# rbesenczi/newMSM

Measured on AMD Instinct MI355X. Metric: label-cost evals/sec, higher is better.
Workload: dtype f64; 1 GPU; pairwise sulc (D=1) unary label-cost table, ico6 data grid / ico4 control grid, 19 labels, 48678 evals = 3187573 point samples per step (BASELINE config 2); kind=univariate, simmeasure=correlation, replicas=1

## Files before the change

include/msmhip.h:

```cpp
#ifndef MSMHIP_H
#define MSMHIP_H

#include <stddef.h>
#include <stdint.h>

#ifdef __cplusplus
extern "C" {
#endif

#define MSM_ABI_VERSION 12

#define MSM_OK 0
#define MSM_ERR_INVALID (-1)
#define MSM_ERR_HIP (-2)
#define MSM_ERR_OUTSIDE (-3)
#define MSM_ERR_NOTFOUND (-4)
#define MSM_ERR_NOGPU (-5)
#define MSM_ERR_STATE (-6)
#define MSM_ERR_CAPACITY (-7)
#define MSM_ERR_ROTATION (-8)

#define MSM_RAD 100.0
#define MSM_FOLDING 1e7

typedef struct msm_ctx msm_ctx;
typedef struct msm_mesh msm_mesh;
typedef struct msm_cost msm_cost;

int         msm_abi_version(void);
const char *msm_last_error(void);
int         msm_device_count(void);

int msm_icosphere_counts(int order, int32_t *V, int32_t *T);
int msm_icosphere(int order, double radius, double *xyz, int32_t *tri);
int msm_mesh_adjacency(const int32_t *tri, int32_t V, int32_t T, int32_t *nbr_ptr, int32_t *nbr, int32_t *tid_ptr, int32_t *tid);
int msm_vertex_areas(const double *xyz, const int32_t *tri, int32_t V, int32_t T, double *area);
int msm_resample_anatomy_grid(const double *cp_xyz, int32_t N, const int32_t *cp_tri, int32_t Tc, int32_t levels, double rad, int32_t *Va, int32_t *Ta,
                              double *axyz, int32_t *atri, int32_t *w_ptr, int32_t *w_cp, double *w_val, int32_t *face_ptr, int32_t *face_idx);
int msm_cp_spacings(const double *xyz, const int32_t *tri, int32_t V, int32_t T, double *maxsep, double *mvdmax);
int msm_label_sampling_grid(int sg_order, double max_dist, int abs_is_int, int32_t cap,
                            double *samples, int32_t *nsamples, double *barycentres, int32_t *nbarycentres);
int msm_rescale_sampling_grid(const double *samples, int32_t n, double *scale, double *labels);
int msm_rotation_matrix(const double ci[3], const double index[3], double R[9]);
int msm_cp_rotations(const double centre[3], const double *cp_xyz, int32_t N, double *rot);
int msm_estimate_triplets(const int32_t *tri, int32_t T, int32_t *triplets);
int msm_estimate_pairs(const int32_t *tri, int32_t V, int32_t T, int32_t *pairs);
int msm_octree_signature(const double *xyz, const int32_t *tri, int32_t V, int32_t T, int64_t stats[5], uint64_t *signature);
int msm_ray_table_check(const double *xyz, const int32_t *tri, int32_t V, int32_t T, int32_t nsamples, uint64_t seed, int64_t report[10]);
int msm_ray_hint_check(const double *xyz, const int32_t *tri, int32_t V, int32_t T, int32_t nsamples, uint64_t seed, int64_t report[8], int32_t *cells,
                       int64_t cells_cap);
int msm_ray_cert_check(const double *xyz, const int32_t *tri, int32_t V, int32_t T, int32_t nsamples, uint64_t seed, int64_t report[8], int32_t *cells,
                       int64_t cells_cap);
int msm_ray_table_signature(const double *xyz, const int32_t *tri, int32_t V, int32_t T, uint64_t out[13]);

msm_ctx *msm_ctx_create(int device);
msm_ctx *msm_ctx_create_on_stream(int device, void *hip_stream);
void     msm_ctx_destroy(msm_ctx *ctx);
int      msm_ctx_synchronize(msm_ctx *ctx);
void    *msm_ctx_stream(msm_ctx *ctx);
void     msm_store_release_i64(int64_t *addr, int64_t value);
int64_t  msm_load_acquire_i64(const int64_t *addr);
int64_t  msm_min_acquire_i64(const int64_t *addr, int32_t n);
int      msm_ctx_wait_stream(msm_ctx *ctx, void *hip_stream);
int      msm_ctx_staging_stats(msm_ctx *ctx, int64_t out[4]);
int      msm_ctx_time_queries(msm_ctx *ctx, int enable);
int      msm_ctx_query_kernel_ms(msm_ctx *ctx, double *ms);
int      msm_query_lanes(int64_t n_queries);
void    *msm_host_alloc(msm_ctx *ctx, size_t bytes);
void     msm_host_free(msm_ctx *ctx, void *p);
int      msm_host_register(msm_ctx *ctx, void *p, size_t bytes);

msm_mesh *msm_mesh_create(msm_ctx *ctx, const double *xyz, int32_t V, const int32_t *tri, int32_t T);
void      msm_mesh_destroy(msm_mesh *m);
int       msm_mesh_update_coords(msm_mesh *m, const double *xyz);
int       msm_mesh_get_coords(msm_mesh *m, double *xyz);
int       msm_mesh_set_features(msm_mesh *m, const double *feat, int32_t D);
int       msm_mesh_sizes(const msm_mesh *m, int32_t *V, int32_t *T, int32_t *D);
int       msm_mesh_octree_stats(msm_mesh *m, int64_t stats[5]);
int       msm_mesh_octree_signature(msm_mesh *m, int64_t stats[5], uint64_t *signature);
int       msm_octree_forest_signatures(msm_ctx *ctx, const double *xyz, int32_t V, const int32_t *tri, int32_t T, int32_t B, uint64_t *signatures);
int       msm_mesh_prepare_search(msm_mesh *m, int wait, int32_t *ready);

#define MSM_WEIGHTS_PROJECTED 0
#define MSM_WEIGHTS_RAW 1
int msm_query_triangles(msm_mesh *target, const double *q_xyz, int32_t N, int32_t *tri_id, int32_t *v_id, double *w, int weight_mode);
int msm_closest_vertex(msm_mesh *target, const double *q_xyz, int32_t N, int32_t *v_id);
int msm_adaptive_barycentric_weights(msm_mesh *in_mesh, msm_mesh *new_mesh, const double *excl,
                                     int32_t *row_ptr, int32_t *col, double *val, int64_t cap, int64_t *nnz);
int msm_metric_resample(msm_mesh *in_mesh, const double *data, int32_t D, msm_mesh *new_mesh, const double *excl, double *out, double *excl_out);
int msm_sphere_project_warp(msm_mesh *from, const double *to_xyz, double *sphere_xyz, int32_t N);
int msm_mesh_sphere_project_warp(msm_mesh *sphere, msm_mesh *from, const double *to_xyz);
int msm_barycentric_coords_resample(msm_mesh *from, const double *coords_xyz, const double *q_xyz, int32_t N, double *out_xyz);
int msm_smooth_data(msm_mesh *orig, const double *data, int32_t D, msm_mesh *sphlow, double sigma, const double *excl, double *out, double *excl_out);
int msm_nearest_neighbour(msm_mesh *orig, const double *data, int32_t D, const double *q_xyz, int32_t N, const double *excl, double *out, double *excl_out);
int msm_create_exclusion(const double *data, int32_t D, int32_t V, double thrl, double thru, double *excl);

typedef struct msm_resample_plan msm_resample_plan;
#define MSM_RESAMPLE_ADAP_BARY   0
#define MSM_RESAMPLE_BARYCENTRIC 1
#define MSM_RESAMPLE_NEAREST     2
#define MSM_RESAMPLE_SMOOTH      3
#define MSM_F64 0
#define MSM_F32 1
// ... 256 lines not shown
```

newmsm_amd/_lib.py:

```python
import ctypes as C
import os

_HERE = os.path.dirname(os.path.abspath(__file__))
LIB_PATH = os.environ.get("MSM_LIB_PATH") or os.path.join(_HERE, "libmsmhip.so")

c_dp = C.POINTER(C.c_double)
c_ip = C.POINTER(C.c_int32)
c_lp = C.POINTER(C.c_int64)

MSM_OK = 0
ERR_NAMES = {-1: "MSM_ERR_INVALID", -2: "MSM_ERR_HIP", -3: "MSM_ERR_OUTSIDE", -4: "MSM_ERR_NOTFOUND", -5: "MSM_ERR_NOGPU",
             -6: "MSM_ERR_STATE", -7: "MSM_ERR_CAPACITY", -8: "MSM_ERR_ROTATION"}


class MsmError(RuntimeError):

    def __init__(self, code, message):
        super().__init__("%s (%d): %s" % (ERR_NAMES.get(code, "MSM_ERR"), code, message))
        self.code = code


class GroupParams(C.Structure):
    _fields_ = [("simmeasure", C.c_int32), ("fixnan", C.c_int32), ("lambda_", C.c_double), ("mu", C.c_double),
                ("kappa", C.c_double), ("k_exp", C.c_double), ("rexp", C.c_double), ("range", C.c_double), ("percentile", C.c_double)]


class CostParams(C.Structure):
    _fields_ = [("kind", C.c_int32), ("simmeasure", C.c_int32), ("rmode", C.c_int32), ("reserved", C.c_int32),
                ("lambda_", C.c_double), ("mu", C.c_double), ("kappa", C.c_double), ("k_exp", C.c_double),
                ("rexp", C.c_double), ("range", C.c_double), ("percentile", C.c_double)]


class LevelFeaturesParams(C.Structure):
    _fields_ = [("exclude", C.c_int32), ("intensity", C.c_int32), ("varnorm", C.c_int32), ("reserved", C.c_int32), ("thrl", C.c_double), ("thru", C.c_double)]


_VP = C.c_void_p
SIGNATURES = {
    "msm_abi_version": (C.c_int, []),
    "msm_last_error": (C.c_char_p, []),
    "msm_device_count": (C.c_int, []),
    "msm_icosphere_counts": (C.c_int, [C.c_int, c_ip, c_ip]),
    "msm_icosphere": (C.c_int, [C.c_int, C.c_double, c_dp, c_ip]),
    "msm_mesh_adjacency": (C.c_int, [c_ip, C.c_int32, C.c_int32, c_ip, c_ip, c_ip, c_ip]),
    "msm_vertex_areas": (C.c_int, [c_dp, c_ip, C.c_int32, C.c_int32, c_dp]),
    "msm_resample_anatomy_grid": (C.c_int, [c_dp, C.c_int32, c_ip, C.c_int32, C.c_int32, C.c_double, c_ip, c_ip, c_dp, c_ip, c_ip, c_ip, c_dp, c_ip, c_ip]),
    "msm_cp_spacings": (C.c_int, [c_dp, c_ip, C.c_int32, C.c_int32, c_dp, c_dp]),
    "msm_label_sampling_grid": (C.c_int, [C.c_int, C.c_double, C.c_int, C.c_int32, c_dp, c_ip, c_dp, c_ip]),
    "msm_rescale_sampling_grid": (C.c_int, [c_dp, C.c_int32, c_dp, c_dp]),
    "msm_rotation_matrix": (C.c_int, [c_dp, c_dp, c_dp]),
    "msm_cp_rotations": (C.c_int, [c_dp, c_dp, C.c_int32, c_dp]),
    "msm_estimate_triplets": (C.c_int, [c_ip, C.c_int32, c_ip]),
    "msm_estimate_pairs": (C.c_int, [c_ip, C.c_int32, C.c_int32, c_ip]),
    "msm_octree_signature": (C.c_int, [c_dp, c_ip, C.c_int32, C.c_int32, C.POINTER(C.c_int64), C.POINTER(C.c_uint64)]),
    "msm_ray_table_check": (C.c_int, [c_dp, c_ip, C.c_int32, C.c_int32, C.c_int32, C.c_uint64, C.POINTER(C.c_int64)]),
    "msm_ray_hint_check": (C.c_int, [c_dp, c_ip, C.c_int32, C.c_int32, C.c_int32, C.c_uint64, C.POINTER(C.c_int64), c_ip, C.c_int64]),
    "msm_ray_cert_check": (C.c_int, [c_dp, c_ip, C.c_int32, C.c_int32, C.c_int32, C.c_uint64, C.POINTER(C.c_int64), c_ip, C.c_int64]),
    "msm_ray_table_signature": (C.c_int, [c_dp, c_ip, C.c_int32, C.c_int32, C.POINTER(C.c_uint64)]),
    "msm_ctx_create": (_VP, [C.c_int]),
    "msm_ctx_create_on_stream": (_VP, [C.c_int, _VP]),
    "msm_ctx_destroy": (None, [_VP]),
    "msm_ctx_synchronize": (C.c_int, [_VP]),
    "msm_ctx_stream": (_VP, [_VP]),
    "msm_store_release_i64": (None, [_VP, C.c_int64]),
    "msm_load_acquire_i64": (C.c_int64, [_VP]),
    "msm_min_acquire_i64": (C.c_int64, [_VP, C.c_int32]),
    "msm_ctx_time_queries": (C.c_int, [_VP, C.c_int]),
    "msm_ctx_query_kernel_ms": (C.c_int, [_VP, c_dp]),
    "msm_query_lanes": (C.c_int, [C.c_int64]),
    "msm_group_context": (_VP, [_VP]),
    "msm_ctx_wait_stream": (C.c_int, [_VP, _VP]),
    "msm_ctx_staging_stats": (C.c_int, [_VP, C.POINTER(C.c_int64)]),
    "msm_host_alloc": (_VP, [_VP, C.c_size_t]),
    "msm_host_free": (None, [_VP, _VP]),
    "msm_host_register": (C.c_int, [_VP, _VP, C.c_size_t]),
    "msm_mesh_create": (_VP, [_VP, c_dp, C.c_int32, c_ip, C.c_int32]),
    "msm_mesh_destroy": (None, [_VP]),
    "msm_mesh_update_coords": (C.c_int, [_VP, c_dp]),
    "msm_mesh_get_coords": (C.c_int, [_VP, c_dp]),
    "msm_mesh_set_features": (C.c_int, [_VP, c_dp, C.c_int32]),
    "msm_mesh_sizes": (C.c_int, [_VP, c_ip, c_ip, c_ip]),
    "msm_mesh_octree_stats": (C.c_int, [_VP, c_lp]),
    "msm_mesh_octree_signature": (C.c_int, [_VP, c_lp, C.POINTER(C.c_uint64)]),
    "msm_octree_forest_signatures": (C.c_int, [_VP, c_dp, C.c_int32, c_ip, C.c_int32, C.c_int32, C.POINTER(C.c_uint64)]),
    "msm_query_triangles": (C.c_int, [_VP, c_dp, C.c_int32, c_ip, c_ip, c_dp, C.c_int]),
    "msm_closest_vertex": (C.c_int, [_VP, c_dp, C.c_int32, c_ip]),
    "msm_adaptive_barycentric_weights": (C.c_int, [_VP, _VP, c_dp, c_ip, c_ip, c_dp, C.c_int64, c_lp]),
    "msm_metric_resample": (C.c_int, [_VP, c_dp, C.c_int32, _VP, c_dp, c_dp, c_dp]),
    "msm_create_exclusion": (C.c_int, [c_dp, C.c_int32, C.c_int32, C.c_double, C.c_double, c_dp]),
    "msm_resample_plan_create": (_VP, [_VP, _VP, C.c_int, c_dp]),
    "msm_resample_plan_create_smooth": (_VP, [_VP, _VP, C.c_double, c_dp]),
    "msm_resample_plan_divisors": (C.c_int, [_VP, c_dp]),
    "msm_resample_plan_destroy": (None, [_VP]),
    "msm_resample_plan_sizes": (C.c_int, [_VP, c_ip, c_ip, c_lp, c_ip]),
    "msm_resample_plan_weights": (C.c_int, [_VP, c_ip, c_ip, c_dp, C.c_int64]),
    "msm_resample_plan_apply": (C.c_int, [_VP, _VP, C.c_int, C.c_int64, _VP, c_dp]),
    "msm_resample_plan_apply_dev": (C.c_int, [_VP, _VP, C.c_int, C.c_int64, _VP]),
    "msm_resample_plan_apply_labels": (C.c_int, [_VP, c_ip, C.c_int64, C.c_int32, c_ip]),
    "msm_sphere_project_warp": (C.c_int, [_VP, c_dp, c_dp, C.c_int32]),
    "msm_mesh_sphere_project_warp": (C.c_int, [_VP, _VP, c_dp]),
    "msm_barycentric_coords_resample": (C.c_int, [_VP, c_dp, c_dp, C.c_int32, c_dp]),
    "msm_smooth_data": (C.c_int, [_VP, c_dp, C.c_int32, _VP, C.c_double, c_dp, c_dp, c_dp]),
    "msm_mesh_unfold": (C.c_int, [_VP, C.c_double, c_ip, c_ip]),
    "msm_mesh_prepare_search": (C.c_int, [_VP, C.c_int, c_ip]),
    "msm_variance_normalise": (C.c_int, [c_dp, C.c_int32, C.c_int32, c_dp]),
    "msm_histogram_match": (C.c_int, [_VP, C.c_int32, C.c_int32, C.c_int32, c_dp, c_dp, C.c_int32, C.c_int32, c_dp, c_dp, C.c_int32, c_dp]),
    "msm_level_features": (C.c_int, [_VP, C.c_int32, C.POINTER(_VP), C.POINTER(c_dp), C.c_int32, c_dp, C.POINTER(LevelFeaturesParams), c_dp, c_dp]),
    "msm_mcmc_optimise": (C.c_int, [c_dp, c_dp, c_ip, C.c_int32, C.c_int32, C.c_int32, C.c_double, C.c_int32, C.c_uint64, c_ip]),
    "msm_mcmc_optimise_gpu": (C.c_int, [_VP, c_dp, c_dp, c_ip, C.c_int32, C.c_int32, C.c_int32, C.c_double, C.c_int32, C.c_uint64, c_ip]),
# ... 144 lines not shown
```

newmsm_amd/api.py:

```python
import ctypes as C

import numpy as np

from ._lib import CostParams, LevelFeaturesParams, MsmError, c_dp, c_ip, c_lp, check, lib

WEIGHTS_PROJECTED = 0
WEIGHTS_RAW = 1
KINDS = dict(univariate=0, multivariate=1, patchwise=2, ho_univariate=3, ho_multivariate=4)


def _soa(points):
    a = np.ascontiguousarray(np.asarray(points, dtype=np.float64).reshape(-1, 3).T)
    return a, a.ctypes.data_as(c_dp)


def _aos(soa, n):
    return np.ascontiguousarray(np.asarray(soa).reshape(3, n).T)


def _tri_soa(tri):
    a = np.ascontiguousarray(np.asarray(tri, dtype=np.int32).reshape(-1, 3).T)
    return a, a.ctypes.data_as(c_ip)


# ... 63 lines not shown
                                        b.ctypes.data_as(c_dp), C.byref(nb)))
    return np.ascontiguousarray(s[:, : ns.value].T), np.ascontiguousarray(b[:, : nb.value].T)


def rescale_sampling_grid(samples, scale):
    s, ps = _soa(samples)
    n = s.shape[1]
    out = np.zeros((3, n))
    sc = C.c_double(scale)
    check(lib().msm_rescale_sampling_grid(ps, n, C.byref(sc), out.ctypes.data_as(c_dp)))
    return np.ascontiguousarray(out.T), sc.value


def estimate_rotation_matrix(ci, index):
    R = np.zeros(9)
    check(lib().msm_rotation_matrix(_d(ci)[1], _d(index)[1], R.ctypes.data_as(c_dp)))
    return R.reshape(3, 3)


def cp_rotations(centre, cp_xyz):
    x, px = _soa(cp_xyz)
    rot = np.zeros((x.shape[1], 9))
    check(lib().msm_cp_rotations(_d(centre)[1], px, x.shape[1], rot.ctypes.data_as(c_dp)))
    return rot


def octree_signature(xyz, tri):
    x, px = _soa(xyz)
    t, pt = _tri_soa(tri)
    stats = (C.c_int64 * 5)()
    sig = C.c_uint64(0)
    check(lib().msm_octree_signature(px, pt, x.shape[1], t.shape[1], stats, C.byref(sig)))
    return dict(nodes=stats[0], leaves=stats[1], depth=stats[2], refs=stats[3], max_leaf=stats[4]), sig.value


def ray_table_check(xyz, tri, nsamples=20000, seed=1):
    x, px = _soa(xyz)
    t, pt = _tri_soa(tri)
    rep = (C.c_int64 * 10)()
    check(lib().msm_ray_table_check(px, pt, x.shape[1], t.shape[1], nsamples, seed, rep))
    return dict(points=rep[0], by_float=rep[1], by_fp64=rep[2], open=rep[3], violations=rep[4], unusable=rep[5], with_exclusions=rep[6], simple=bool(rep[7]), boxes_checked=rep[8], refused_by_boxes=rep[9])


def ray_hint_check(xyz, tri, nsamples=20000, seed=1, return_cells=False):
    x, px = _soa(xyz)
    t, pt = _tri_soa(tri)
    rep = (C.c_int64 * 8)()
    cells = np.zeros((6 * 512 * 512, 4), dtype=np.int32) if return_cells else None
    check(lib().msm_ray_hint_check(px, pt, x.shape[1], t.shape[1], nsamples, seed, rep, cells.ctypes.data_as(c_ip) if return_cells else None, cells.size if return_cells else 0))
    out = dict(points=rep[0], hinted=rep[1], unhinted=rep[2], listed=rep[3], cells_changed=rep[4], cells=rep[5], cells_with_more=rep[6], subcells=rep[7])
    if return_cells:
        out["cell_array"] = cells[: rep[5]].copy()
    return out


def ray_cert_check(xyz, tri, nsamples=20000, seed=1, return_cells=False):
    x, px = _soa(xyz)
    t, pt = _tri_soa(tri)
    rep = (C.c_int64 * 8)()
    cells = np.zeros((6 * 512 * 512, 4), dtype=np.int32) if return_cells else None
    check(lib().msm_ray_cert_check(px, pt, x.shape[1], t.shape[1], nsamples, seed, rep, cells.ctypes.data_as(c_ip) if return_cells else None, cells.size if return_cells else 0))
    out = dict(points=rep[0], certified_points=rep[1], fp64_failures=rep[2], reference_disagrees=rep[3], subcells=rep[4], certified_subcells=rep[5], cells=rep[6], placed=rep[7])
    if return_cells:
        out["cell_array"] = cells[: rep[6]].copy()
    return out


def ray_table_signature(xyz, tri):
    x, px = _soa(xyz)
    t, pt = _tri_soa(tri)
    out = (C.c_uint64 * 13)()
    check(lib().msm_ray_table_signature(px, pt, x.shape[1], t.shape[1], out))
    names = ("G", "simple", "certs", "cells", "edges", "more", "excl", "r2lo_bits", "r2hi_bits", "cell_hash", "edge_hash", "more_hash", "excl_hash")
    return dict(zip(names, (int(v) for v in out)))


def estimate_triplets(tri):
    t, pt = _tri_soa(tri)
    out = np.zeros((t.shape[1], 3), dtype=np.int32)
    check(lib().msm_estimate_triplets(pt, t.shape[1], out.ctypes.data_as(c_ip)))
    return out


def estimate_pairs(tri, V):
    t, pt = _tri_soa(tri)
    n = lib().msm_estimate_pairs(pt, V, t.shape[1], None)
    if n < 0:
        check(n)
    out = np.zeros((n, 2), dtype=np.int32)
    lib().msm_estimate_pairs(pt, V, t.shape[1], out.ctypes.data_as(c_ip))
    return out


class Context:

    def __init__(self, device=0, stream=None):
        L = lib()
        self.h = L.msm_ctx_create(device) if stream is None else L.msm_ctx_create_on_stream(device, C.c_void_p(stream))
        if not self.h:
            raise MsmError(-5, L.msm_last_error().decode())
        self.device = device

    def synchronize(self):
        check(lib().msm_ctx_synchronize(self.h))

    @property
# ... 1217 lines not shown
```

newmsm_amd/csrc/ray_table_check.cpp:

```cpp
#include <algorithm>
#include <cmath>
#include <cstring>

#include "ray_table.hpp"
#include "search_device.hpp"

namespace msm {

namespace {

struct TableUnderTest {
    const char *hook = "";
    const double *xyz = nullptr;
    const int32_t *tri = nullptr;
    int V = 0, T = 0;
    FlatOctree o;
    DevTree dt{};
    uint64_t rs = 0;
    std::vector<int> hits;

    int build(const char *hook_, const double *xyz_, const int32_t *tri_, int32_t V_, int32_t T_, int32_t nsamples, uint64_t seed, int64_t *report, int nreport) {
        hook = hook_, xyz = xyz_, tri = tri_, V = V_, T = T_;
        if (!xyz || !tri || !report || V <= 0 || T <= 0 || nsamples < 0) return fail(MSM_ERR_INVALID, "%s: bad arguments", hook);
        for (int64_t i = 0; i < 3 * (int64_t)T; ++i)
// ... 140 lines not shown
    return MSM_OK;
}

extern "C" int msm_ray_hint_check(const double *xyz, const int32_t *tri, int32_t V, int32_t T, int32_t nsamples, uint64_t seed, int64_t report[8], int32_t *cells,
                                  int64_t cells_cap) {
    using namespace msm;
    TableUnderTest u;
    MSM_TRY(u.build("msm_ray_hint_check", xyz, tri, V, T, nsamples, seed, report, 8));
    const FlatOctree &o = u.o;
    const DevTree &dt = u.dt;
    report[7] = kRayHintK;
    if (o.rays.G <= 0) return MSM_OK;
    const size_t ncell = o.rays.cell.size();
    report[5] = (int64_t)ncell;
    MSM_TRY(u.copy_cells(cells, cells_cap));
    for (size_t c = 0; c < ncell; ++c) {
        const int4 raw = o.rays.cell[c], ids = ray_cell_ids(raw);
        if (ids.x >= 0 && ids.w < -1) ++report[6];
        const int stored[4] = {ids.x, ids.y, ids.z, ids.w};
        bool same = true;
        for (int k = 0; k < 4; ++k) same = same && stored[k] < T && (stored[k] >= -1 || (k == 3 && -2 - stored[k] < (int)o.rays.more.size()));
        for (int su = 0; su < kRayHintK && same; ++su)
            for (int sv = 0; sv < kRayHintK && same; ++sv) {
                const int h = ray_cell_hint(raw, su, sv);
                const int4 d = ray_cell_first(raw, h);
                const int got[4] = {d.x, d.y, d.z, d.w};
                same = got[0] == stored[h] && (stored[0] < 0 || got[0] >= 0);
                for (int k = 0, j = 1; k < 4; ++k)
                    if (k != h) same = same && got[j++] == stored[k];
            }
        if (!same) ++report[4];
    }
    for (int it = 0; it < nsamples; ++it) {
        const V3 p = scale(normalized(u.random_direction()), kRad);
        ++report[0];
        const std::vector<int> &hits = u.first_pass(p);
        if (hits.size() != 1) continue;
        const int answer = hits[0];
        float fx, fy, fz;
        size_t at;
        int su, sv;
        if (!ray_cell_at(dt, p, fx, fy, fz, at, su, sv)) continue;
        const int4 first = ray_cell_of(dt, p, fx, fy, fz), ids = ray_cell_ids(o.rays.cell[at]);
        if (first.x == answer) ++report[1];
        if (ids.x == answer) ++report[2];
        int4 more = make_int4(ids.w, -1, -1, -1);
        if (ids.x >= 0 && ids.w < -1) more = o.rays.more[-2 - ids.w];
        const int list[7] = {ids.x, ids.y, ids.z, more.x, more.y, more.z, more.w};
        for (int k = 0; k < 7; ++k)
            if (list[k] == answer) {
                ++report[3];
                break;
            }
    }
    return MSM_OK;
}

extern "C" int msm_ray_cert_check(const double *xyz, const int32_t *tri, int32_t V, int32_t T, int32_t nsamples, uint64_t seed, int64_t report[8], int32_t *cells,
                                  int64_t cells_cap) {
    using namespace msm;
    TableUnderTest u;
    MSM_TRY(u.build("msm_ray_cert_check", xyz, tri, V, T, nsamples, seed, report, 8));
    const FlatOctree &o = u.o;
    const DevTree &dt = u.dt;
    if (o.rays.G <= 0) return MSM_OK;
    const size_t ncell = o.rays.cell.size();
    report[6] = (int64_t)ncell;
    MSM_TRY(u.copy_cells(cells, cells_cap));
    for (size_t c = 0; c < ncell; ++c)
        for (int su = 0; su < kRayHintK; ++su)
            for (int sv = 0; sv < kRayHintK; ++sv) {
                ++report[4];
                if (ray_cell_cert(o.rays.cell[c], su, sv)) ++report[5];
            }
    auto rnd = [&]() { return u.rnd(); };
    const int G = o.rays.G;
    auto on_face = [&](int f, double uu, double v) {
        const int a = f >> 1;
        double comp[3];
        comp[a] = (f & 1) ? -1.0 : 1.0, comp[(a + 1) % 3] = uu, comp[(a + 2) % 3] = v;
        return mk(comp[0], comp[1], comp[2]);
    };
    auto check = [&](V3 p) {
        p = scale(normalized(p), kRad);
        ++report[0];
        float fx, fy, fz;
        bool cert;
        const int4 first = ray_cell_of(dt, p, fx, fy, fz, cert);
        if (!cert) return;
        ++report[1];
        const int t = first.x;
        if (t < 0 || t >= T) {
            ++report[2], ++report[3];
            return;
        }
        if (!ray_accepts_fp64(u.vert(t, 0), u.vert(t, 1), u.vert(t, 2), p, norm(p), (double)o.rays.edge[3 * (size_t)t].w - kRayFloatAllowance + 1e-12)) ++report[2];
        const std::vector<int> &hits = u.first_pass(p);
        if (!(hits.size() == 1 && hits[0] == t)) ++report[3];
    };
    for (int it = 0; it < nsamples; ++it) check(u.random_direction());
    const int64_t before = report[0];
    const double cellw = 2.0 / G;
    auto nudge = [&]() { return rnd() < 0.2 ? 0.0 : (rnd() < 0.5 ? -1.0 : 1.0) * 1e-6 * rnd() * cellw; };
    auto border = [&](bool cell_border) {
        const int i = (int)(rnd() * G) % G, s = cell_border ? 0 : 1 + (int)(rnd() * (kRayHintK - 1)) % std::max(1, kRayHintK - 1);
        return -1 + 2.0 * (i + (double)s / kRayHintK) / G + nudge();
// ... 46 lines not shown
```

newmsm_amd/csrc/unary_kernels.hip:

```cpp
#include "search_device.hpp"
#include "similarity_device.hpp"
#include "unary.hpp"

namespace msm {

namespace {

constexpr int kDeferred = 1 << 20;
constexpr unsigned kInvalidPair = 0xffffffffu;

__device__ __forceinline__ void raise_status(int *status, int code) { atomicMin(status, code); }

struct SamplesArgs {
    DevTree tree;
    const double *tfeat;
    int tD;
    int N, L;
    const double *rnl;
    const double *src;
    int Nsrc;
    const int *pptr, *pidx;
    const int *order;
    int pmax;
    int nsplit;
    double *tval;
    int *stri;
    double *sw3;
    unsigned long long *fix_list;
    double *fix_pt;
    unsigned int *fix_cnt;
    const unsigned int *fix_off;
    const double *sfeat;
    const double *cfw;
    const double *absw;
    int simmeasure;
    double percentile;
    double *U;
    int *redo_list;
    unsigned int *redo_count;
    int *status;
};

__device__ __forceinline__ int fast_div(int s, int P, float invP) {
    int q = (int)((float)s * invP);
    if (q * P > s) --q;
    else if ((q + 1) * P <= s) ++q;
    return q;
}

__device__ __forceinline__ double emit_sample(const SamplesArgs &a, size_t g, const V3 &p, int t) {
    const TriRec &r = a.tree.rec[t];
    double wa, wb, wc;
    area_weights(rec_v0(r), rec_v1(r), rec_v2(r), p, wa, wb, wc);
    if (a.tval) {
        const double v = wa * a.tfeat[(size_t)r.id[0] * a.tD] + wb * a.tfeat[(size_t)r.id[1] * a.tD] + wc * a.tfeat[(size_t)r.id[2] * a.tD];
        a.tval[g] = v;
        return v;
    } else {
        a.stri[g] = t;
        a.sw3[3 * g] = wa;
        a.sw3[3 * g + 1] = wb;
        a.sw3[3 * g + 2] = wc;
    }
    return 0.0;
}

__device__ __forceinline__ void emit_failure(const SamplesArgs &a, size_t g, int code) {
    raise_status(a.status, code);
    const double nan = __longlong_as_double(0x7ff8000000000000ll);
    if (a.tval) {
        a.tval[g] = nan;
    } else {
        a.stri[g] = code;
        a.sw3[3 * g] = a.sw3[3 * g + 1] = a.sw3[3 * g + 2] = nan;
    }
}

}

__global__ __launch_bounds__(256) void k_unary_samples(SamplesArgs a) {
    extern __shared__ __align__(16) double lds[];
    double *sx = lds, *sy = sx + a.pmax, *sz = sy + a.pmax;
    double *sA = sz + a.pmax;
    double *sR = sA + 2 * a.pmax;
    double *sT = sR + 9 * a.L;
    unsigned *queue = reinterpret_cast<unsigned *>(sT + (size_t)unary_labels_per_workgroup(a.L, a.nsplit) * a.pmax);
    int *nin = reinterpret_cast<int *>(queue + kQueueCap);
    int *win = nin + kChunk;
    __shared__ int s_qn, s_ndefer;
    const int tid = threadIdx.x, lane = tid & 63;

    {
        int at, l_beg, l_end;
        if (!unary_workgroup_share(blockIdx.x, a.N, a.L, a.nsplit, at, l_beg, l_end)) return;
        const int node = a.order[at];
        const int beg = a.pptr[node], P = a.pptr[node + 1] - beg;
        const size_t gbase = (size_t)a.L * beg;
        for (int i = tid; i < P; i += 256) {
            const int s = a.pidx[beg + i];
            sx[i] = a.src[s];
            sy[i] = a.src[a.Nsrc + s];
            sz[i] = a.src[2 * a.Nsrc + s];
            if (a.U) sA[i] = a.sfeat[s];
        }
        for (int k = tid; k < 9 * a.L; k += 256) sR[k] = a.rnl[(size_t)node * a.L * 9 + k];
        if (tid == 0) s_ndefer = 0;
        const int sbeg = l_beg * P, send = l_end * P;
        const float invP = 1.0f / (float)max(P, 1);

        for (int base = sbeg; base < send; base += kChunk) {
            const int nchunk = min(kChunk, send - base);
            for (int k = tid; k < kChunk; k += 256) nin[k] = 0;
            if (tid == 0) s_qn = 0;
            __syncthreads();

            for (int r0 = 0; r0 < nchunk; r0 += 256) {
                const int sl = r0 + tid;
                unsigned long long pm = 0ull;
                int lbeg = 0;
                bool defer = false;
                if (sl < nchunk) {
                    const int s = base + sl;
                    const int l = fast_div(s, P, invP), i = s - l * P;
                    const V3 p = rotate(sR + 9 * l, mk(sx[i], sy[i], sz[i]));
                    if (outside_root(p)) {
                        nin[sl] = -1;
                    } else {
                        int sub;
                        const int4 leaf = locate_leaf(a.tree, p, sub);
                        lbeg = leaf.y;
// ... 65 lines not shown
                const V3 p = rotate(sR + 9 * l, mk(sx[i], sy[i], sz[i]));
                V3 mp;
                if (inside_test(a.tree.rec[t], p, mp)) {
                    win[sl] = t;
                    atomicAdd(&nin[sl], 1);
                }
            }
            __syncthreads();

            for (int sl = tid; sl < nchunk; sl += 256) {
                const int s = base + sl;
                const int n = nin[sl];
                if (n == 1) {
                    const int l = fast_div(s, P, invP), i = s - l * P;
                    const V3 p = rotate(sR + 9 * l, mk(sx[i], sy[i], sz[i]));
                    const double v = emit_sample(a, gbase + s, p, win[sl]);
                    if (a.U) sT[(l - l_beg) * a.pmax + i] = v;
                } else if (n < 0) {
                    emit_failure(a, gbase + s, MSM_ERR_OUTSIDE);
                    atomicAdd(&s_ndefer, 1);
                } else {
                    atomicAdd(&s_ndefer, 1);
                    const int seg = blockIdx.x % kFixSegs;
                    const unsigned slot = a.fix_off[seg] + atomicAdd(&a.fix_cnt[kCntStride * (1 + seg)], 1u);
                    if (slot < a.fix_off[seg + 1]) {
                        const int l = fast_div(s, P, invP), i = s - l * P;
                        const V3 p = rotate(sR + 9 * l, mk(sx[i], sy[i], sz[i]));
                        a.fix_list[slot] = gbase + (unsigned long long)s;
                        a.fix_pt[3 * (size_t)slot] = p.x;
                        a.fix_pt[3 * (size_t)slot + 1] = p.y;
                        a.fix_pt[3 * (size_t)slot + 2] = p.z;
                    } else {
                        raise_status(a.status, MSM_ERR_CAPACITY);
                    }
                }
            }
            __syncthreads();
        }
        if (a.U) {
            __syncthreads();
            if (s_ndefer == 0) {
                const double absw = a.absw[node];
                for (int l = l_beg + (tid >> 6); l < l_end; l += 4) {
                    const double cost = patch_dice(sA, sT + (l - l_beg) * a.pmax, P, lane, a.simmeasure, a.percentile);
                    if (lane == 0) a.U[(size_t)l * a.N + node] = absw * cost;
                }
            } else if (tid == 0) {
                a.redo_list[atomicAdd(a.redo_count, 1u)] = node;
            }
        }
    }
}

__global__ __launch_bounds__(256) __attribute__((amdgpu_waves_per_eu(7))) void k_unary_rays(SamplesArgs a) {
    extern __shared__ __align__(16) double lds[];
    double *sx = lds, *sy = sx + a.pmax, *sz = sy + a.pmax, *sR = sz + a.pmax;
    const int tid = threadIdx.x, lane = tid & 63;
    const int per = (a.N + 7) >> 3;
    const int slots = 8 * per;
    const int part = blockIdx.x / slots, slot = blockIdx.x - part * slots;
    const int at = (slot & 7) * per + (slot >> 3);
    if (at >= a.N) return;
    const int node = a.order[at];
    const int lper = (a.L + a.nsplit - 1) / a.nsplit;
    const int l_beg = part * lper, l_end = min(a.L, l_beg + lper);
    if (l_beg >= l_end) return;
    const int beg = a.pptr[node], P = a.pptr[node + 1] - beg;
    const size_t gbase = (size_t)a.L * beg;
    for (int i = tid; i < P; i += 256) {
        const int s = a.pidx[beg + i];
        sx[i] = a.src[s];
        sy[i] = a.src[a.Nsrc + s];
        sz[i] = a.src[2 * a.Nsrc + s];
    }
    for (int k = 9 * l_beg + tid; k < 9 * l_end; k += 256) sR[k] = a.rnl[(size_t)node * a.L * 9 + k];
    const int sbeg = l_beg * P, send = l_end * P;
    const float invP = 1.0f / (float)max(P, 1);
    int *sleft = reinterpret_cast<int *>(sR + 9 * a.L);
    __shared__ int s_nleft;
    __shared__ unsigned s_base;
    if (tid == 0) s_nleft = 0;
    __syncthreads();
    for (int s0 = sbeg; s0 < send; s0 += 256) {
        const int s = s0 + tid;
        const bool act = s < send;
        bool done = false;
        V3 p = mk(0.0, 0.0, 0.0);
        float fx = 0.f, fy = 0.f, fz = 0.f;
        int4 c = make_int4(-1, -1, -1, -1);
        bool cert = false;
        if (act) {
            const int l = fast_div(s, P, invP), i = s - l * P;
            p = rotate(sR + 9 * l, mk(sx[i], sy[i], sz[i]));
            c = ray_cell_of(a.tree, p, fx, fy, fz, cert);
        }
        if (act) {
            if (c.x >= 0) {
                const float4 *rec = a.tree.ray_tri + (size_t)kRayPieces * c.x;
                const double2 *dv = reinterpret_cast<const double2 *>(rec + 3);
                int t = c.x;
                int excl = -1;
                bool retry = false;
#ifdef __HIP_DEVICE_COMPILE__
                typedef float v4f __attribute__((ext_vector_type(4)));
                v4f q0, q1, q2;
                asm volatile("" : "=v"(q0), "=v"(q1), "=v"(q2));
                if (!cert) {
                    const v4f *rq = reinterpret_cast<const v4f *>(rec);
                    q0 = rq[0], q1 = rq[1], q2 = rq[2];
                }
                double2 d0 = dv[0], d1 = dv[1], d2 = dv[2], d3 = dv[3], d4 = dv[4], d5 = dv[5];
                if (!cert) {
                    asm volatile("" : "+v"(q0), "+v"(q1), "+v"(q2));
                    const float4 e0 = make_float4(q0.x, q0.y, q0.z, q0.w), e1 = make_float4(q1.x, q1.y, q1.z, q1.w), e2 = make_float4(q2.x, q2.y, q2.z, q2.w);
#else
                double2 d0 = dv[0], d1 = dv[1], d2 = dv[2], d3 = dv[3], d4 = dv[4], d5 = dv[5];
                if (!cert) {
                    const float4 e0 = rec[0], e1 = rec[1], e2 = rec[2];
#endif
                    excl = __float_as_int(e1.w);
                    retry = !ray_accepts(e0, e1, e2, fx, fy, fz);
                }
                if (retry) {
                    t = -1;
                    int4 mo = make_int4(c.w, -1, -1, -1);
                    if (c.w < -1) mo = a.tree.ray_more[-2 - c.w];
#pragma unroll 1
                    for (int k = 0; k < 6 && t < 0; ++k) {
                        const int ck = k == 0 ? c.y : (k == 1 ? c.z : (k == 2 ? mo.x : (k == 3 ? mo.y : (k == 4 ? mo.z : mo.w))));
                        if (ck < 0) break;
                        const float4 *r2 = a.tree.ray_tri + (size_t)kRayPieces * ck;
                        const float4 g0 = r2[0], g1 = r2[1], g2 = r2[2];
                        if (ray_accepts(g0, g1, g2, fx, fy, fz)) {
                            t = ck;
                            excl = __float_as_int(g1.w);
                        }
                    }
                    if (t >= 0) {
                        dv = reinterpret_cast<const double2 *>(a.tree.ray_tri + (size_t)kRayPieces * t + 3);
                        d0 = dv[0], d1 = dv[1], d2 = dv[2], d3 = dv[3], d4 = dv[4], d5 = dv[5];
                    }
                }
                if (t >= 0 && excl >= 0 && !ray_vouches(a.tree, make_float4(0.f, 0.f, 0.f, __int_as_float(excl)), p)) t = -1;
                if (t >= 0) {
                    double wa, wb, wc;
                    area_weights(mk(d0.x, d0.y, d1.x), mk(d1.y, d2.x, d2.y), mk(d3.x, d3.y, d4.x), p, wa, wb, wc);
                    const size_t g = gbase + s;
                    if (a.tval) {
                        a.tval[g] = wa * d4.y + wb * d5.x + wc * d5.y;
                    } else {
                        a.stri[g] = t;
                        a.sw3[3 * g] = wa;
                        a.sw3[3 * g + 1] = wb;
                        a.sw3[3 * g + 2] = wc;
                    }
                    done = true;
                }
            }
        }
        const bool left = act && !done;
        const unsigned long long bal = __ballot(left);
        if (bal) {
            const int leader = __ffsll((long long)bal) - 1;
            int base = 0;
            if (lane == leader) base = atomicAdd(&s_nleft, __popcll(bal));
            base = __shfl(base, leader, 64);
            if (left) sleft[base + __popcll(bal & ((1ull << lane) - 1ull))] = s;
        }
    }
    __syncthreads();
    const int nleft = s_nleft;
    if (nleft > 0) {
        const int seg = blockIdx.x % kFixSegs;
        if (tid == 0) s_base = a.fix_off[seg] + atomicAdd(&a.fix_cnt[kCntStride * (1 + seg)], (unsigned)nleft);
        __syncthreads();
        const unsigned base = s_base, end = a.fix_off[seg + 1];
        for (int j = tid; j < nleft; j += 256) {
            if (base + j < end) {
                const int s = sleft[j];
                const int l = fast_div(s, P, invP), i = s - l * P;
                const V3 p = rotate(sR + 9 * l, mk(sx[i], sy[i], sz[i]));
                a.fix_list[base + j] = gbase + (unsigned long long)s;
                a.fix_pt[3 * (size_t)(base + j)] = p.x;
                a.fix_pt[3 * (size_t)(base + j) + 1] = p.y;
                a.fix_pt[3 * (size_t)(base + j) + 2] = p.z;
            } else {
                raise_status(a.status, MSM_ERR_CAPACITY);
            }
        }
    }
}

__global__ __launch_bounds__(256) void k_unary_fixup(SamplesArgs a) {
    __shared__ unsigned s_pre[kFixSegs + 1];
    if (threadIdx.x < kFixSegs) {
        const int seg = threadIdx.x;
        const unsigned cnt = min(a.fix_cnt[kCntStride * (1 + seg)], a.fix_off[seg + 1] - a.fix_off[seg]);
        unsigned incl = cnt;
#pragma unroll
        for (int off = 1; off < 64; off <<= 1) {
            const unsigned up = __shfl_up(incl, off, 64);
            if (seg >= off) incl += up;
        }
        s_pre[seg + 1] = incl;
        if (seg == 0) s_pre[0] = 0;
    }
    __syncthreads();
    const unsigned n = s_pre[kFixSegs];
    const int lane = threadIdx.x & 63, sub = lane & 7, grp = lane >> 3;
    const unsigned per_block = 256 / 8, stride = gridDim.x * per_block;
    for (unsigned j0 = blockIdx.x * per_block + (threadIdx.x >> 6) * 8; j0 < n; j0 += stride) {
        const unsigned j = j0 + grp;
        const bool valid = j < n;
        V3 p = mk(0.0, 0.0, 0.0);
        size_t g = 0;
        if (valid) {
            int seg = 0;
#pragma unroll
            for (int step = kFixSegs / 2; step > 0; step >>= 1)
                if (s_pre[seg + step] <= j) seg += step;
            const size_t slot = a.fix_off[seg] + (j - s_pre[seg]);
            g = (size_t)a.fix_list[slot];
            p = mk(a.fix_pt[3 * slot], a.fix_pt[3 * slot + 1], a.fix_pt[3 * slot + 2]);
        }
        const int found = group8_find(a.tree, valid, p, lane);
        if (valid && sub == 0) {
            const int t = found == kGroupUndecided ? find_closest_triangle(a.tree, p) : found;
            if (t < 0) emit_failure(a, g, t);
            else emit_sample(a, g, p, t);
        }
    }
}

int launch_samples(msm_ctx *ctx, const UnaryLaunch &u, const UnaryPlan &plan, const UnaryWeightsScratch *w, bool fused_reduction) {
    if (u.tree.nnodes <= 0 || !u.tree.mask) return fail(MSM_ERR_STATE, "target search structure missing");
    if (u.ntri >= (1 << kTriBits)) return fail(MSM_ERR_CAPACITY, "target mesh has %d triangles; the sample queue packs ids in %d bits", u.ntri, kTriBits);
    const bool rays = plan.sampler == MSM_SAMPLER_RAYS;
    SamplesArgs a;
    a.tree = u.tree;
    a.tfeat = u.tfeat;
    a.tD = u.D > 0 ? u.D : 1;
    a.N = u.N;
    a.L = u.L;
    a.rnl = u.rnl;
// ... 40 lines not shown
```

Baseline: 392.2 million evals/s.

## Resolve ray-cell retry candidates cooperatively across 8-lane teams in wave

Restructures the retry path in the ray-based point location kernel. The first alternate candidate (c.y) is tested per lane, and only the plane data is loaded. Lanes still unresolved are then served in rounds, where 8-lane groups each take one pending lane and test its remaining candidates in parallel, so the serial per-lane loop is replaced with ballots and shuffles. Triangle payload is loaded once after acceptance, and an mbcnt-based prefix count replaces the popcount mask. It also adds a host-side diagnostic that reports at which list depth the correct triangle is found. The risk is extra shuffle and ballot overhead and register pressure when few lanes need retries.

```diff
diff --git a/include/msmhip.h b/include/msmhip.h
--- a/include/msmhip.h
+++ b/include/msmhip.h
@@ -49,6 +49,7 @@
 int msm_ray_table_check(const double *xyz, const int32_t *tri, int32_t V, int32_t T, int32_t nsamples, uint64_t seed, int64_t report[10]);
 int msm_ray_hint_check(const double *xyz, const int32_t *tri, int32_t V, int32_t T, int32_t nsamples, uint64_t seed, int64_t report[8], int32_t *cells,
                        int64_t cells_cap);
+int msm_ray_depth_check(const double *xyz, const int32_t *tri, int32_t V, int32_t T, int32_t nsamples, uint64_t seed, int64_t report[8]);
 int msm_ray_cert_check(const double *xyz, const int32_t *tri, int32_t V, int32_t T, int32_t nsamples, uint64_t seed, int64_t report[8], int32_t *cells,
                        int64_t cells_cap);
 int msm_ray_table_signature(const double *xyz, const int32_t *tri, int32_t V, int32_t T, uint64_t out[13]);
diff --git a/newmsm_amd/_lib.py b/newmsm_amd/_lib.py
--- a/newmsm_amd/_lib.py
+++ b/newmsm_amd/_lib.py
@@ -55,6 +55,7 @@
     "msm_octree_signature": (C.c_int, [c_dp, c_ip, C.c_int32, C.c_int32, C.POINTER(C.c_int64), C.POINTER(C.c_uint64)]),
     "msm_ray_table_check": (C.c_int, [c_dp, c_ip, C.c_int32, C.c_int32, C.c_int32, C.c_uint64, C.POINTER(C.c_int64)]),
     "msm_ray_hint_check": (C.c_int, [c_dp, c_ip, C.c_int32, C.c_int32, C.c_int32, C.c_uint64, C.POINTER(C.c_int64), c_ip, C.c_int64]),
+    "msm_ray_depth_check": (C.c_int, [c_dp, c_ip, C.c_int32, C.c_int32, C.c_int32, C.c_uint64, C.POINTER(C.c_int64)]),
     "msm_ray_cert_check": (C.c_int, [c_dp, c_ip, C.c_int32, C.c_int32, C.c_int32, C.c_uint64, C.POINTER(C.c_int64), c_ip, C.c_int64]),
     "msm_ray_table_signature": (C.c_int, [c_dp, c_ip, C.c_int32, C.c_int32, C.POINTER(C.c_uint64)]),
     "msm_ctx_create": (_VP, [C.c_int]),
diff --git a/newmsm_amd/api.py b/newmsm_amd/api.py
--- a/newmsm_amd/api.py
+++ b/newmsm_amd/api.py
@@ -139,6 +139,14 @@
     if return_cells:
         out["cell_array"] = cells[: rep[5]].copy()
     return out
+
+
+def ray_depth_check(xyz, tri, nsamples=20000, seed=1):
+    x, px = _soa(xyz)
+    t, pt = _tri_soa(tri)
+    rep = (C.c_int64 * 8)()
+    check(lib().msm_ray_depth_check(px, pt, x.shape[1], t.shape[1], nsamples, seed, rep))
+    return dict(points=rep[0], at=[int(rep[k]) for k in range(1, 7)], unlisted=rep[7])
 
 
 def ray_cert_check(xyz, tri, nsamples=20000, seed=1, return_cells=False):
diff --git a/newmsm_amd/csrc/ray_table_check.cpp b/newmsm_amd/csrc/ray_table_check.cpp
--- a/newmsm_amd/csrc/ray_table_check.cpp
+++ b/newmsm_amd/csrc/ray_table_check.cpp
@@ -216,6 +216,36 @@
                 ++report[3];
                 break;
             }
+    }
+    return MSM_OK;
+}
+
+extern "C" int msm_ray_depth_check(const double *xyz, const int32_t *tri, int32_t V, int32_t T, int32_t nsamples, uint64_t seed, int64_t report[8]) {
+    using namespace msm;
+    TableUnderTest u;
+    MSM_TRY(u.build("msm_ray_depth_check", xyz, tri, V, T, nsamples, seed, report, 8));
+    const FlatOctree &o = u.o;
+    const DevTree &dt = u.dt;
+    if (o.rays.G <= 0) return MSM_OK;
+    for (int it = 0; it < nsamples; ++it) {
+        const V3 p = scale(normalized(u.random_direction()), kRad);
+        ++report[0];
+        const std::vector<int> &hits = u.first_pass(p);
+        if (hits.size() != 1) continue;
+        const int answer = hits[0];
+        float fx, fy, fz;
+        const int4 c = ray_cell_of(dt, p, fx, fy, fz);
+        if (c.x < 0) continue;
+        int4 more = make_int4(c.w, -1, -1, -1);
+        if (c.w < -1) more = o.rays.more[-2 - c.w];
+        const int list[7] = {c.x, c.y, c.z, more.x, more.y, more.z, more.w};
+        int at = 7;
+        for (int k = 0; k < 7 && list[k] >= 0; ++k)
+            if (list[k] == answer) {
+                at = k;
+                break;
+            }
+        ++report[at == 7 ? 7 : 1 + std::min(at, 5)];
     }
     return MSM_OK;
 }
diff --git a/newmsm_amd/csrc/unary_kernels.hip b/newmsm_amd/csrc/unary_kernels.hip
--- a/newmsm_amd/csrc/unary_kernels.hip
+++ b/newmsm_amd/csrc/unary_kernels.hip
@@ -76,6 +76,19 @@
     }
 }
 
+#ifndef MSM_RAY_RETRY
+#define MSM_RAY_RETRY 3
+#endif
+static_assert(MSM_RAY_RETRY >= 0 && MSM_RAY_RETRY <= 3, "0: rolled loop, 1: round A + loop, 2: round A + team round, 3: round A (planes only) + team round");
+
+__device__ __forceinline__ int set_below(unsigned long long m) {
+#ifdef __HIP_DEVICE_COMPILE__
+    return (int)__builtin_amdgcn_mbcnt_hi((unsigned)(m >> 32), __builtin_amdgcn_mbcnt_lo((unsigned)m, 0u));
+#else
+    return 0;
+#endif
+}
+
 }
 
 __global__ __launch_bounds__(256) void k_unary_samples(SamplesArgs a) {
@@ -247,6 +260,22 @@
     }
 }
 
+#define RAY_EMIT_ACCEPTED()                                                                                                                      \
+    if (t >= 0 && excl >= 0 && !ray_vouches(a.tree, make_float4(0.f, 0.f, 0.f, __int_as_float(excl)), p)) t = -1;  \
+    if (t >= 0) {                                                                                                                                \
+        double wa, wb, wc;                                                                                                                       \
+        area_weights(mk(d0.x, d0.y, d1.x), mk(d1.y, d2.x, d2.y), mk(d3.x, d3.y, d4.x), p, wa, wb, wc);                                           \
+        const size_t g = gbase + s;                                                                                                              \
+        if (a.tval) {                                                                                                                            \
+            a.tval[g] = wa * d4.y + wb * d5.x + wc * d5.y;                                                                                       \
+        } else {                                                                                                                                 \
+            a.stri[g] = t;                                                                                                                       \
+            a.sw3[3 * g] = wa;                                                                                                                   \
+            a.sw3[3 * g + 1] = wb;                                                                                                               \
+            a.sw3[3 * g + 2] = wc;                                                                                                               \
+        }                                                                                                                                        \
+        done = true;                                                                                                                             \
+    }
 __global__ __launch_bounds__(256) __attribute__((amdgpu_waves_per_eu(7))) void k_unary_rays(SamplesArgs a) {
     extern __shared__ __align__(16) double lds[];
     double *sx = lds, *sy = sx + a.pmax, *sz = sy + a.pmax, *sR = sz + a.pmax;
@@ -289,12 +318,39 @@
             p = rotate(sR + 9 * l, mk(sx[i], sy[i], sz[i]));
             c = ray_cell_of(a.tree, p, fx, fy, fz, cert);
         }
+#if MSM_RAY_RETRY >= 2
+        int t = -1;
+        int excl = -1;
+        double2 d0, d1, d2, d3, d4, d5;
+        bool pend = false;
+        bool got = false;
+        int4 mo;
+#ifdef __HIP_DEVICE_COMPILE__
+        {
+            typedef double v2d __attribute__((ext_vector_type(2)));
+            typedef int v4i __attribute__((ext_vector_type(4)));
+            v2d u0, u1, u2, u3, u4, u5;
+            v4i um;
+            asm volatile("" : "=v"(u0), "=v"(u1), "=v"(u2), "=v"(u3), "=v"(u4), "=v"(u5), "=v"(um));
+            d0 = make_double2(u0.x, u0.y), d1 = make_double2(u1.x, u1.y), d2 = make_double2(u2.x, u2.y);
+            d3 = make_double2(u3.x, u3.y), d4 = make_double2(u4.x, u4.y), d5 = make_double2(u5.x, u5.y);
+            mo = make_int4(um.x, um.y, um.z, um.w);
+        }
+#else
+        d0 = d1 = d2 = d3 = d4 = d5 = make_double2(0.0, 0.0);
+        mo = make_int4(-1, -1, -1, -1);
+#endif
+#endif
         if (act) {
             if (c.x >= 0) {
                 const float4 *rec = a.tree.ray_tri + (size_t)kRayPieces * c.x;
                 const double2 *dv = reinterpret_cast<const double2 *>(rec + 3);
-                int t = c.x;
+#if MSM_RAY_RETRY < 2
+                int t;
                 int excl = -1;
+                double2 d0, d1, d2, d3, d4, d5;
+#endif
+                t = c.x;
                 bool retry = false;
 #ifdef __HIP_DEVICE_COMPILE__
                 typedef float v4f __attribute__((ext_vector_type(4)));
@@ -304,12 +360,12 @@
                     const v4f *rq = reinterpret_cast<const v4f *>(rec);
                     q0 = rq[0], q1 = rq[1], q2 = rq[2];
                 }
-                double2 d0 = dv[0], d1 = dv[1], d2 = dv[2], d3 = dv[3], d4 = dv[4], d5 = dv[5];
+                d0 = dv[0], d1 = dv[1], d2 = dv[2], d3 = dv[3], d4 = dv[4], d5 = dv[5];
                 if (!cert) {
                     asm volatile("" : "+v"(q0), "+v"(q1), "+v"(q2));
                     const float4 e0 = make_float4(q0.x, q0.y, q0.z, q0.w), e1 = make_float4(q1.x, q1.y, q1.z, q1.w), e2 = make_float4(q2.x, q2.y, q2.z, q2.w);
 #else
-                double2 d0 = dv[0], d1 = dv[1], d2 = dv[2], d3 = dv[3], d4 = dv[4], d5 = dv[5];
+                d0 = dv[0], d1 = dv[1], d2 = dv[2], d3 = dv[3], d4 = dv[4], d5 = dv[5];
                 if (!cert) {
                     const float4 e0 = rec[0], e1 = rec[1], e2 = rec[2];
 #endif
@@ -318,10 +374,40 @@
                 }
                 if (retry) {
                     t = -1;
+#if MSM_RAY_RETRY >= 2
+                    mo = make_int4(c.w, -1, -1, -1);
+#else
                     int4 mo = make_int4(c.w, -1, -1, -1);
+                    bool reload = true;
+#endif
+#if MSM_RAY_RETRY >= 1
+                    if (c.y >= 0) {
+                        const float4 *r2 = a.tree.ray_tri + (size_t)kRayPieces * c.y;
+                        const float4 g0 = r2[0], g1 = r2[1], g2 = r2[2];
+#if MSM_RAY_RETRY != 3
+                        dv = reinterpret_cast<const double2 *>(r2 + 3);
+                        d0 = dv[0], d1 = dv[1], d2 = dv[2], d3 = dv[3], d4 = dv[4], d5 = dv[5];
+#endif
+                        if (c.w < -1) mo = a.tree.ray_more[-2 - c.w];
+                        if (ray_accepts(g0, g1, g2, fx, fy, fz)) {
+                            t = c.y;
+                            excl = __float_as_int(g1.w);
+#if MSM_RAY_RETRY == 3
+                            got = true;
+#endif
+                        }
+#if MSM_RAY_RETRY >= 2
+                        pend = t < 0 && c.z >= 0;
+#else
+                        reload = t < 0;
+#endif
+                    }
+#else
                     if (c.w < -1) mo = a.tree.ray_more[-2 - c.w];
+#endif
+#if MSM_RAY_RETRY < 2
 #pragma unroll 1
-                    for (int k = 0; k < 6 && t < 0; ++k) {
+                    for (int k = MSM_RAY_RETRY; k < 6 && t < 0; ++k) {
                         const int ck = k == 0 ? c.y : (k == 1 ? c.z : (k == 2 ? mo.x : (k == 3 ? mo.y : (k == 4 ? mo.z : mo.w))));
                         if (ck < 0) break;
                         const float4 *r2 = a.tree.ray_tri + (size_t)kRayPieces * ck;
@@ -331,28 +417,59 @@
                             excl = __float_as_int(g1.w);
                         }
                     }
-                    if (t >= 0) {
+                    if (t >= 0 && reload) {
                         dv = reinterpret_cast<const double2 *>(a.tree.ray_tri + (size_t)kRayPieces * t + 3);
                         d0 = dv[0], d1 = dv[1], d2 = dv[2], d3 = dv[3], d4 = dv[4], d5 = dv[5];
                     }
-                }
-                if (t >= 0 && excl >= 0 && !ray_vouches(a.tree, make_float4(0.f, 0.f, 0.f, __int_as_float(excl)), p)) t = -1;
-                if (t >= 0) {
-                    double wa, wb, wc;
-                    area_weights(mk(d0.x, d0.y, d1.x), mk(d1.y, d2.x, d2.y), mk(d3.x, d3.y, d4.x), p, wa, wb, wc);
-                    const size_t g = gbase + s;
-                    if (a.tval) {
-                        a.tval[g] = wa * d4.y + wb * d5.x + wc * d5.y;
-                    } else {
-                        a.stri[g] = t;
-                        a.sw3[3 * g] = wa;
-                        a.sw3[3 * g + 1] = wb;
-                        a.sw3[3 * g + 2] = wc;
-                    }
-                    done = true;
-                }
-            }
-        }
+#endif
+                }
+#if MSM_RAY_RETRY < 2
+                RAY_EMIT_ACCEPTED();
+#endif
+            }
+        }
+#if MSM_RAY_RETRY >= 2
+        for (unsigned long long want = __ballot(pend); want != 0ull;) {
+            const int grp = lane >> 3, sub = lane & 7;
+            int owner = -1;
+            unsigned long long rest = want;
+#pragma unroll
+            for (int i = 0; i < 8; ++i) {
+                const int o = __ffsll((long long)rest) - 1;
+                if (grp == i) owner = o;
+                rest &= rest - 1ull;
+            }
+            const int from = owner < 0 ? lane : owner;
+            const float ox = __shfl(fx, from, 64), oy = __shfl(fy, from, 64), oz = __shfl(fz, from, 64);
+            const int k0 = __shfl(c.z, from, 64), k1 = __shfl(mo.x, from, 64), k2 = __shfl(mo.y, from, 64), k3 = __shfl(mo.z, from, 64), k4 = __shfl(mo.w, from, 64);
+            int ck = sub == 0 ? k0 : (sub == 1 ? k1 : (sub == 2 ? k2 : (sub == 3 ? k3 : (sub == 4 ? k4 : -1))));
+            if (owner < 0) ck = -1;
+            bool ok = false;
+            int ex = -1;
+            if (ck >= 0) {
+                const float4 *r2 = a.tree.ray_tri + (size_t)kRayPieces * ck;
+                const float4 g0 = r2[0], g1 = r2[1], g2 = r2[2];
+                ok = ray_accepts(g0, g1, g2, ox, oy, oz);
+                ex = __float_as_int(g1.w);
+            }
+            const unsigned long long hit = __ballot(ok);
+            const int rank = set_below(want);
+            const bool served = pend && rank < 8;
+            const unsigned byte = served ? (unsigned)(hit >> (8 * rank)) & 0xffu : 0u;
+            const int helper = byte ? 8 * rank + __ffs((int)byte) - 1 : lane;
+            const int hck = __shfl(ck, helper, 64), hex = __shfl(ex, helper, 64);
+            if (byte) t = hck, excl = hex, got = true;
+            if (served) pend = false;
+            want = rest;
+        }
+        if (got) {
+            const double2 *dv = reinterpret_cast<const double2 *>(a.tree.ray_tri + (size_t)kRayPieces * t + 3);
+            d0 = dv[0], d1 = dv[1], d2 = dv[2], d3 = dv[3], d4 = dv[4], d5 = dv[5];
+        }
+        if (act) {
+            RAY_EMIT_ACCEPTED();
+        }
+#endif
         const bool left = act && !done;
         const unsigned long long bal = __ballot(left);
         if (bal) {
@@ -360,7 +477,7 @@
             int base = 0;
             if (lane == leader) base = atomicAdd(&s_nleft, __popcll(bal));
             base = __shfl(base, leader, 64);
-            if (left) sleft[base + __popcll(bal & ((1ull << lane) - 1ull))] = s;
+            if (left) sleft[base + set_below(bal)] = s;
         }
     }
     __syncthreads();
@@ -385,6 +502,7 @@
         }
     }
 }
+#undef RAY_EMIT_ACCEPTED
 
 __global__ __launch_bounds__(256) void k_unary_fixup(SamplesArgs a) {
     __shared__ unsigned s_pre[kFixSegs + 1];
```

New measurement: 396.8 million evals/s (median of 6 runs). 1.2% higher.
